# KUIS-AI-Tekalp-Research-Group/video-compression

Measured on AMD Instinct MI355X. Metric: frames/sec + bpp/PSNR on UVG 1080p GOP-8, 1/2/4/8 MI355X, higher is better.
Workload: dtype f32; 1 GPU; LHBDC 1080p GOP-8 inference, single lambda: 7 B-frames per GOP via Model.forward, 4 independent GOP(s) per GPU per step, hierarchy levels batched across them; gop=8, resolution=1920x1080, precision=fp32, parallelism=gop-shard x1, launch=hip-graph per GOP pass

## Files before the change

include/vc_hip.h:

```cpp
#ifndef VC_HIP_H
#define VC_HIP_H

#include <stddef.h>
#include <stdint.h>

#ifdef __cplusplus
extern "C" {
#endif

#define VC_OK 0
#define VC_EINVAL (-1)
#define VC_ELAUNCH (-2)
#define VC_ENOMEM (-3)
#define VC_EDATA (-4)

typedef void *vc_stream;

typedef struct {
    float *p;
    int n, h, w, c;
    long long sn, sh, sw;
} vc_view;

const char *vc_version(void);
// ... 115 lines not shown
int vc_gc_forward(vc_stream s, vc_view y, vc_view scales, vc_view means, const float *in_gain,
                  const float *out_gain, vc_view y_hat, double *bits_partial, int bits_slots,
                  const float *sym_src_p, int32_t *symbols, int32_t *indexes, const float *scale_table,
                  int n_scales, float *likelihoods);
int vc_gc_indexes(vc_stream s, vc_view scales, const float *scale_table, int n_scales, int32_t *indexes);
int vc_refine_scales(vc_stream s, vc_view scales, vc_view in, const float *w_oihw, const float *bias, const float *scale_table,
                     int n_scales, float rel_eps, int *counter);
int vc_gc_dequant(vc_stream s, const int32_t *symbols, vc_view means, const float *out_gain, vc_view y_hat);
typedef struct vc_refine_layer {
    vc_view in;
    const float *w_oihw;
    const float *bias;
    int k, stride, c0;
} vc_refine_layer;
int vc_refine_y_symbols(vc_stream s, vc_view y, vc_refine_layer y_layer, vc_view means, vc_refine_layer mu_layer, float eps,
                        int32_t *symbols, vc_view y_hat, const float *out_gain, int *counter);
int vc_refine_z_symbols(vc_stream s, vc_view z, vc_refine_layer z_layer, const float *eb_params, const float *in_gain, float eps,
                        int32_t *symbols, vc_view z_hat, const float *out_gain, int *counter);
int vc_bits_reduce(vc_stream s, const double *partial, int slots, int count, double *out);
int vc_bits_slots(void);
int vc_psnr_uint8(vc_stream s, const float *a_chw, const float *b_chw, int channels, int H, int W, int h, int w,
                  double *scratch, int slots, double *psnr_out);
size_t vc_msssim_workspace_bytes(int n, int channels, int h, int w);
int vc_msssim(vc_stream s, const float *a, const float *b, int n, int channels, int H, int W, int h, int w,
              long long image_pitch, int quantize, void *workspace, size_t workspace_bytes, double *terms_out,
              double *msssim_out);

int vc_pmf_to_quantized_cdf(const float *pmf, int n, int precision, uint32_t *cdf_out );
size_t vc_rans_bound(size_t count);
long long vc_rans_encode_with_indexes(const int32_t *symbols, const int32_t *indexes, size_t count,
                                      const int32_t *cdfs, int n_tables, int cdf_stride, const int32_t *cdf_sizes,
                                      const int32_t *offsets, uint8_t *out, size_t out_cap);
int vc_rans_decode_with_indexes(const uint8_t *data, size_t nbytes, const int32_t *indexes, size_t count,
                                const int32_t *cdfs, int n_tables, int cdf_stride, const int32_t *cdf_sizes,
                                const int32_t *offsets, int32_t *symbols_out);
int vc_rans_decode_stream(const uint8_t *data, size_t nbytes, uint64_t *state, const int32_t *indexes, size_t count,
                          const int32_t *cdfs, int n_tables, int cdf_stride, const int32_t *cdf_sizes,
                          const int32_t *offsets, int32_t *symbols_out);

int vc_gdn(vc_stream s, vc_view x, const float *gamma_packed, const float *beta_packed, int inverse, vc_view res ,
           vc_view out);
int vc_spynet_level(vc_stream s, vc_view first, vc_view second, vc_view flow_coarse, vc_view feat8, vc_view up2);
int vc_pool(vc_stream s, vc_view in, vc_view out, int k, float scale);
int vc_upsample(vc_stream s, vc_view in, vc_view out, int factor, int align_corners, float scale);
int vc_pad(vc_stream s, vc_view in, vc_view out);
int vc_blend(vc_stream s, vc_view fwbw, vc_view mask, vc_view cur, vc_view pred, vc_view resid);
int vc_factorized_bits(vc_stream s, vc_view z, const float *params, const float *in_gain, const float *out_gain,
                       vc_view z_hat, int32_t *symbols, double *bits_partial, int bits_slots, float *likelihoods);
int vc_gaussian_symbols(vc_stream s, vc_view y, vc_view scales, vc_view means, const float *in_gain,
                        const float *out_gain, vc_view y_hat, double *bits_partial, int bits_slots,
                        const float *sym_src_p, int32_t *symbols, int32_t *indexes, const float *scale_table,
                        int n_scales, float *likelihoods);

#ifdef __cplusplus
}
#endif
#endif
```

video-compression_amd/csrc/conv_api.hip:

```cpp
#include <stdlib.h>
#include <string.h>
#include "conv_mfma.h"

static inline int cfg_nt(int cfg) { return cfg == VC_CFG_N4 ? 4 : (cfg == VC_CFG_N16 ? 16 : 32); }
static inline int cfg_ks(int cfg) { return cfg == VC_CFG_N4 ? 4 : (cfg == VC_CFG_N16 ? 16 : 8); }
static inline int cfg_bn(int cfg)
{
    switch (cfg) {
    case VC_CFG_N128:
    case VC_CFG_N128B: return 128;
    case VC_CFG_N64: return 64;
    case VC_CFG_N32:
    case VC_CFG_N32T16: return 32;
    case VC_CFG_N4: return 4;
    default: return 16;
    }
}
static inline int round_up(int a, int b) { return (a + b - 1) / b * b; }

extern "C" int vc_conv_select_cfg(int cout, int cin, int k, int stride)
{
    (void)cin;
    int cfg;
    if (cout <= 4 && stride == 1 && (k == 3 || k == 5 || k == 7)) cfg = VC_CFG_N4;
// ... 197 lines not shown
    if (a.res_f16 && (!f16 || !d->res || !((d->cfg & 0xff) == VC_CFG_PWS || (d->cfg & 0xff) == VC_CFG_DMA))) return VC_EINVAL;
    a.res_first = (d->cfg & VC_CFG_RES_FIRST) ? 1 : 0;
    if (a.res_first && (!d->res || d->epi != VC_EPI_NONE || d->act == VC_ACT_SIGMOID || d->act == VC_ACT_CLAMP01)) return VC_EINVAL;
    a.cin_pad = round_up(a.Cin, f16 ? 2 * ck : ck);
    const int cfg0 = d->cfg & 0xff;
    const int th = (cfg0 == VC_CFG_N32T16) ? 16 : 8, tw = (cfg0 == VC_CFG_N4) ? 64 : 32;
    a.tiles_x = (a.Wo + tw - 1) / tw;
    a.tiles_y = (a.Ho + th - 1) / th;
    int cfg = d->cfg & 0xff;
    const bool exact = (d->cfg & VC_CFG_EXACT) != 0;
    while (!exact && (cfg == VC_CFG_N128 || cfg == VC_CFG_N64) &&
           (long long)a.tiles_x * a.tiles_y * a.N * (round_up(a.Cout, cfg_bn(cfg)) / cfg_bn(cfg)) < 512 &&
           vc_conv_chunk(cfg + 1, k, st, d->in.c) == ck)
        ++cfg;
    const int bn = cfg_bn(cfg);
    a.nblks = round_up(a.Cout, bn) / bn;
    a.total_blocks = a.tiles_x * a.tiles_y * a.nblks * a.N;
    {
        static const int band = [] { const char *e = getenv("VC_TILE_BAND"); const int v = e ? atoi(e) : 8; return v >= 1 ? v : 8; }();
        a.tile_band = band;
    }
    a.act = d->act; a.slope = d->slope;
    a.epi = d->epi; a.in_xform = d->in_xform; a.out_mode = d->out_mode;
    a.vec4 = ((a.Cin % 4) == 0 && (a.in_sw % 4) == 0 && (a.in_sh % 4) == 0 && (a.in_sn % 4) == 0 &&
              ((uintptr_t)a.in % 16) == 0) ? 1 : 0;
    if (a.in_f16)
        a.vec4 = ((a.Cin % 8) == 0 && (a.in_sw % 8) == 0 && (a.in_sh % 8) == 0 && (a.in_sn % 8) == 0 &&
                  ((uintptr_t)a.in % 16) == 0) ? 1 : 0;
    {
        auto ok = [](const void *ptr, long long sn, long long sh, long long sw) {
            return !ptr || (((uintptr_t)ptr % 16) == 0 && (sn % 4) == 0 && (sh % 4) == 0 && (sw % 4) == 0);
        };
        const int cgrp = (d->out_mode == VC_OUT_PIXELSHUFFLE2) ? (a.Cout >> 2) : a.Cout;
        a.vec_out = (cgrp % 4) == 0 && (a.out_sp3 ? ((uintptr_t)a.out % 16) == 0 : ok(a.out, a.out_sn, a.out_sh, a.out_sw)) &&
                    (a.res_sp3 ? ((uintptr_t)a.res % 8) == 0 : ok(a.res, a.res_sn, a.res_sh, a.res_sw)) &&
                    ok(a.mul, a.mul_sn, a.mul_sh, a.mul_sw) && ok(a.chscale, 0, 0, 0);
    }
    if (a.total_blocks <= 0) return VC_EINVAL;
    if (a.out_sp3 && !a.vec_out) return VC_EINVAL;
    if (f16 && !a.vec4) return VC_EINVAL;
    hipStream_t stream = as_stream(s);
    if (cfg == VC_CFG_PW) {
        if (!conv_pw_eligible(a, k, st, f16)) return VC_EINVAL;
        return conv_dispatch_pw(stream, a, f16);
    }
    if (cfg == VC_CFG_PWS) {
        if (!conv_pws_eligible(a, k, st, f16)) return VC_EINVAL;
        return conv_dispatch_pws(stream, a, f16);
    }
    if (cfg == VC_CFG_SPLIT)
        return conv_dispatch_split(stream, a, k, st);
    if (cfg == VC_CFG_DMA)
        return conv_dispatch_dma(stream, a, k, st, f16);
    switch (k) {
    case 1: return f16 ? conv_dispatch_k1_f16(stream, a, st, cfg, ck) : conv_dispatch_k1_f32(stream, a, st, cfg, ck);
    case 3: return f16 ? conv_dispatch_k3_f16(stream, a, st, cfg, ck) : conv_dispatch_k3_f32(stream, a, st, cfg, ck);
    case 5: return f16 ? conv_dispatch_k5_f16(stream, a, st, cfg, ck) : conv_dispatch_k5_f32(stream, a, st, cfg, ck);
    case 7: return f16 ? conv_dispatch_k7_f16(stream, a, st, cfg, ck) : conv_dispatch_k7_f32(stream, a, st, cfg, ck);
    }
    return VC_EINVAL;
}

#ifdef VC_STAMPS
extern "C" int vc_debug_read_stamps(unsigned long long *out8)
{
    if (hipDeviceSynchronize() != hipSuccess) return VC_ELAUNCH;
    if (hipMemcpyFromSymbol(out8, HIP_SYMBOL(g_vc_stamps), 8 * sizeof(unsigned long long)) != hipSuccess) return VC_ELAUNCH;
    unsigned long long zero[8] = {0};
    if (hipMemcpyToSymbol(HIP_SYMBOL(g_vc_stamps), zero, sizeof(zero)) != hipSuccess) return VC_ELAUNCH;
    return VC_OK;
}
extern "C" int vc_debug_set_skip(int mask)
{
    if (hipDeviceSynchronize() != hipSuccess) return VC_ELAUNCH;
    return hipMemcpyToSymbol(HIP_SYMBOL(g_vc_skip), &mask, sizeof(mask)) == hipSuccess ? VC_OK : VC_ELAUNCH;
}
#endif
```

video-compression_amd/csrc/conv_mfma.h:

```cpp
#pragma once
#include "common.h"

#include <type_traits>
#include <utility>

__device__ __forceinline__ void vc_tile_xy(int t, int tiles_x, int tiles_y, int band_rows, int &tx, int &ty)
{
    const int per_band = band_rows * tiles_x;
    const int band = t / per_band, r = t - band * per_band;
    const int rows = min(band_rows, tiles_y - band * band_rows);
    tx = r / rows;
    ty = band * band_rows + (r - tx * rows);
}

template <int I, int N, class F> __device__ __forceinline__ void static_for(F &&f)
{
    if constexpr (I < N) {
        f(std::integral_constant<int, I>{});
        static_for<I + 1, N>(std::forward<F>(f));
    }
}

#ifdef VC_STAMPS
__device__ unsigned long long g_vc_stamps[8];
// ... 710 lines not shown
    } else {
        conv_epilogue<C, F16>(p, acc, nblk, wm, wn, lane, oy0, ox0, img);
    }
    VC_T(t_end);
    VC_ACC(4, t_end, t_loop_end);
    VC_ACC(5, t_end, t_start);
    VC_ACC(6, 1ull, 0ull);
}

template <int KH, int KW, int S, int CK, class C, bool F16 = false, bool BLDS = false> int launch_conv(hipStream_t st, const ConvArgs &a)
{
    typedef ConvGeom<KH, KW, S, CK, C> G;
    const size_t lds_bytes = (G::LDS_FLOATS + 4) * sizeof(float) +
                             (BLDS ? (size_t)KH * KW * (a.cin_pad / G::KS) * 64 : 0);
    auto kern = conv_mfma_kernel<KH, KW, S, CK, C, F16, BLDS>;
    static vc_lds_raised raised;
    if (!vc_raise_lds_limit(reinterpret_cast<const void *>(kern), lds_bytes, raised)) return VC_ELAUNCH;
    hipLaunchKernelGGL(kern, dim3(a.total_blocks), dim3(256), lds_bytes, st, a);
    return hipGetLastError() == hipSuccess ? VC_OK : VC_ELAUNCH;
}

#ifdef VC_TU_F16
template <int KH, int KW, int S, int CK, class C> int launch_conv_p(hipStream_t st, const ConvArgs &a)
{
    return launch_conv<KH, KW, S, CK, C, VC_TU_F16 != 0>(st, a);
}
template <int KH, int KW, int S, int CK> int launch_conv_n4(hipStream_t st, const ConvArgs &a)
{
#if VC_TU_F16
    return VC_EINVAL;
#else
    const char *force = getenv("VC_N4_GLOBAL_WEIGHTS");
    if ((size_t)KH * KW * (a.cin_pad / 4) * 64 <= 32 * 1024 && !(force && force[0] == '1'))
        return launch_conv<KH, KW, S, CK, CfgN4, false, true>(st, a);
    return launch_conv<KH, KW, S, CK, CfgN4, false>(st, a);
#endif
}
#if VC_TU_F16
#define VC_DISPATCH(k) conv_dispatch_##k##_f16
#else
#define VC_DISPATCH(k) conv_dispatch_##k##_f32
#endif
#endif

#define VC_DECLARE_DISPATCH(k)                                                             \
    int conv_dispatch_##k##_f32(hipStream_t st, const ConvArgs &a, int stride, int cfg, int ck); \
    int conv_dispatch_##k##_f16(hipStream_t st, const ConvArgs &a, int stride, int cfg, int ck);
bool conv_pw_eligible(const ConvArgs &a, int k, int stride, bool f16);
bool conv_pws_eligible(const ConvArgs &a, int k, int stride, bool f16);
int conv_dispatch_pws(hipStream_t st, const ConvArgs &a, bool f16);
int conv_dispatch_pw(hipStream_t st, const ConvArgs &a, bool f16);
int conv_dispatch_dma(hipStream_t st, ConvArgs a, int k, int stride, bool f16);
int conv_dispatch_split(hipStream_t st, ConvArgs a, int k, int stride);
VC_DECLARE_DISPATCH(k1)
VC_DECLARE_DISPATCH(k3)
VC_DECLARE_DISPATCH(k5)
VC_DECLARE_DISPATCH(k7)
```

video-compression_amd/vcamd/hip.py:

```python
import contextlib
import ctypes
import os

import numpy as np
import torch

_PKG_DIR = os.path.dirname(os.path.dirname(os.path.abspath(__file__)))
LIB_PATH = os.environ.get("VC_HIP_LIB") or os.path.join(_PKG_DIR, "libvc_hip.so")

VC_OK = 0
ABI_VERSION = 6
ACT_NONE, ACT_RELU, ACT_LRELU, ACT_SIGMOID, ACT_CLAMP01 = 0, 1, 2, 3, 4
EPI_NONE, EPI_GDN, EPI_IGDN = 0, 1, 2
IN_NONE, IN_SQUARE = 0, 1
OUT_PLAIN, OUT_PIXELSHUFFLE2 = 0, 1
WARP_W1, WARP_W2, WARP_W3 = 1, 2, 3
EB_PARAMS_PER_CHANNEL = 60

_ERR = {-1: "VC_EINVAL (bad argument / unsupported shape)", -2: "VC_ELAUNCH (HIP launch failure)",
        -3: "VC_ENOMEM", -4: "VC_EDATA (corrupt bitstream / degenerate pmf)"}


class VcError(RuntimeError):
    pass
# ... 101 lines not shown
    sig("vc_split3", ci, vp, View, vp, cll)
    sig("vc_split3_pad", ci, vp, View, vp, cll, ci)
    sig("vc_nchw_to_nhwc", ci, vp, vp, View)
    sig("vc_nhwc_to_nchw", ci, vp, View, vp)
    sig("vc_u8hwc_to_f32nchw_pad", ci, vp, vp, ci, ci, vp, ci, ci)
    sig("vc_f32nchw_to_u8hwc", ci, vp, vp, ci, ci, vp, ci, ci)
    sig("vc_avgpool_reflectpad", ci, vp, View, View, ci, cf)
    sig("vc_maxpool2", ci, vp, View, View)
    sig("vc_maxpool2_sp3", ci, vp, vp, cll, ci, ci, ci, ci, vp, cll)
    sig("vc_avgpool2_sp3", ci, vp, vp, cll, ci, ci, ci, ci, cf, vp, cll, View)
    sig("vc_upsample_bilinear_sp3", ci, vp, View, vp, cll, ci, ci, cf)
    sig("vc_upsample_bilinear", ci, vp, View, View, ci, ci, cf)
    sig("vc_axpby", ci, vp, View, View, View, cf, cf)
    sig("vc_clamp01", ci, vp, View, View)
    sig("vc_channel_scale", ci, vp, View, vp, View)
    sig("vc_warp", ci, vp, ci, View, View, View)
    sig("vc_spynet_preprocess", ci, vp, vp, View)
    sig("vc_spynet_level_input", ci, vp, View, View, View, View, View)
    sig("vc_spynet_level_input_sp3", ci, vp, View, View, View, vp, View)
    sig("vc_lhbdc_blend", ci, vp, View, View, View, View, View)
    sig("vc_flex_blend", ci, vp, View, View, View, View, View, View)
    sig("vc_flex_motion_split", ci, vp, View, View, View, cf)
    sig("vc_quantize_mask", ci, vp, View, View, vp, ci, ci)
    sig("vc_deform_pack_weights", ci, vp, ci, ci, ci, vp)
    sig("vc_deform_conv2d", ci, vp, View, View, View, vp, vp, ci, View)
    sig("vc_offset_diversity", ci, vp, View, View, View, View, View, View, cf, vp, vp, ci, View)
    sig("vc_offset_diversity_hx", ci, vp, View, View, View, View, View, View, cf, vp, vp, ci, View)
    sig("vc_to_half", ci, vp, View, vp)
    sig("vc_offset_diversity_hxp", ci, vp, View, View, View, View, View, View, cf, vp, vp, ci, View)
    sig("vc_to_half_planar", ci, vp, View, ci, vp)
    sig("vc_attention_gate", ci, vp, View, View, View, View)
    sig("vc_sse_clamp01", ci, vp, View, View, vp, ci)
    sig("vc_select_flow", ci, vp, vp, ci, ctypes.c_double, ctypes.POINTER(View), View, vp)
    sig("vc_eb_forward", ci, vp, View, vp, vp, vp, View, vp, vp, ci, vp)
    sig("vc_eb_dequant", ci, vp, vp, vp, vp, View)
    sig("vc_gc_forward", ci, vp, View, View, View, vp, vp, View, vp, ci, vp, vp, vp, vp, ci, vp)
    sig("vc_gc_indexes", ci, vp, View, vp, ci, vp)
    sig("vc_refine_scales", ci, vp, View, View, vp, vp, vp, ci, cf, vp)
    sig("vc_gc_dequant", ci, vp, vp, View, vp, View)
    sig("vc_refine_y_symbols", ci, vp, View, RefineLayer, View, RefineLayer, cf, vp, View, vp, vp)
    sig("vc_refine_z_symbols", ci, vp, View, RefineLayer, vp, vp, cf, vp, View, vp, vp)
    sig("vc_bits_reduce", ci, vp, vp, ci, ci, vp)
    sig("vc_bits_slots", ci)
    sig("vc_psnr_uint8", ci, vp, vp, vp, ci, ci, ci, ci, ci, vp, ci, vp)
    sig("vc_msssim_workspace_bytes", sz, ci, ci, ci, ci)
    sig("vc_msssim", ci, vp, vp, vp, ci, ci, ci, ci, ci, ci, cll, ci, vp, sz, vp, vp)
    sig("vc_gdn", ci, vp, View, vp, vp, ci, View, View)
    sig("vc_pad", ci, vp, View, View)
    sig("vc_pmf_to_quantized_cdf", ci, vp, ci, ci, vp)
    sig("vc_rans_bound", sz, sz)
    sig("vc_rans_encode_with_indexes", cll, vp, vp, sz, vp, ci, ci, vp, vp, vp, sz)
    sig("vc_rans_decode_with_indexes", ci, vp, sz, vp, sz, vp, ci, ci, vp, vp, vp)
    sig("vc_rans_decode_stream", ci, vp, sz, vp, vp, sz, vp, ci, ci, vp, vp, vp)
    _lib = L
    return L


EXPORTED_SYMBOLS = [
    "vc_version", "vc_abi_version", "vc_target_arch", "vc_conv_select_cfg", "vc_conv_chunk", "vc_conv_packed_weight_floats",
    "vc_conv_packed_bias_floats", "vc_conv_pack_weights", "vc_conv_packed_weight_bytes_f16",
    "vc_conv_pack_weights_f16", "vc_conv_pack_tail_f16", "vc_conv2d_nhwc", "vc_conv_packed_weight_bytes_split",
    "vc_conv_pack_weights_split", "vc_split3", "vc_split3_pad", "vc_nchw_to_nhwc",
    "vc_nhwc_to_nchw", "vc_u8hwc_to_f32nchw_pad", "vc_f32nchw_to_u8hwc", "vc_avgpool_reflectpad", "vc_maxpool2", "vc_maxpool2_sp3", "vc_avgpool2_sp3", "vc_upsample_bilinear", "vc_upsample_bilinear_sp3", "vc_axpby", "vc_clamp01", "vc_channel_scale", "vc_warp",
    "vc_spynet_preprocess", "vc_spynet_level_input", "vc_spynet_level_input_sp3", "vc_lhbdc_blend", "vc_flex_blend",
    "vc_flex_motion_split", "vc_quantize_mask", "vc_deform_pack_weights", "vc_deform_conv2d", "vc_offset_diversity", "vc_offset_diversity_hx", "vc_to_half", "vc_offset_diversity_hxp", "vc_to_half_planar",
    "vc_attention_gate", "vc_sse_clamp01", "vc_select_flow", "vc_eb_forward", "vc_eb_dequant", "vc_gc_forward", "vc_gc_indexes", "vc_refine_scales",
    "vc_refine_y_symbols", "vc_refine_z_symbols", "vc_gc_dequant", "vc_bits_reduce", "vc_bits_slots", "vc_psnr_uint8", "vc_msssim_workspace_bytes", "vc_msssim", "vc_pmf_to_quantized_cdf", "vc_rans_bound",
    "vc_rans_encode_with_indexes", "vc_rans_decode_with_indexes", "vc_rans_decode_stream",
    "vc_gdn", "vc_spynet_level", "vc_pool", "vc_upsample", "vc_pad", "vc_blend", "vc_factorized_bits", "vc_gaussian_symbols",
]


DEBUG_SYNC = bool(int(os.environ.get("VC_DEBUG_SYNC", "0")))


def check(rc, what):
    if rc != VC_OK:
        raise VcError(f"{what} failed: {_ERR.get(rc, rc)}")
    if DEBUG_SYNC:
        try:
            torch.cuda.synchronize()
        except Exception as e:
            raise VcError(f"device fault during {what}: {e}") from e


def stream():
    return ctypes.c_void_p(torch.cuda.current_stream().cuda_stream)


class T:
    __slots__ = ("buf", "n", "h", "w", "c", "sn", "sh", "sw", "off", "dtype")

    def __init__(self, buf, n, h, w, c, sn, sh, sw, off=0, dtype="f32"):
        self.buf, self.n, self.h, self.w, self.c = buf, n, h, w, c
        self.sn, self.sh, self.sw, self.off, self.dtype = sn, sh, sw, off, dtype

    @staticmethod
    def empty(n, h, w, c, device, dtype="f32"):
        if dtype == "sp3":
            if c % 8:
                raise VcError("a split tensor holds groups of 8 channels")
            return T(torch.empty(n * h * w * c * 3, dtype=torch.int16, device=device), n, h, w, c, c // 8, 0, 0, 0, dtype)
        buf = torch.empty(n * h * w * c, dtype=torch.float16 if dtype == "f16" else torch.float32, device=device)
        return T(buf, n, h, w, c, h * w * c, w * c, c, 0, dtype)

    def channels(self, c0, c1):
        if self.dtype == "sp3":
            if c0 % 8 or c1 % 8:
                raise VcError("a split tensor is sliced in groups of 8 channels")
            return T(self.buf, self.n, self.h, self.w, c1 - c0, self.sn, 0, 0, self.off + c0 // 8, self.dtype)
        return T(self.buf, self.n, self.h, self.w, c1 - c0, self.sn, self.sh, self.sw, self.off + c0, self.dtype)

    def crop(self, h, w):
        if self.dtype == "sp3":
            raise VcError("a split tensor is plane-major: it has no crop window")
        return T(self.buf, self.n, h, w, self.c, self.sn, self.sh, self.sw, self.off, self.dtype)

    def images(self, n0, n1):
        if self.dtype == "sp3":
            return T(self.buf, n1 - n0, self.h, self.w, self.c, self.sn, 0, 0, self.off + n0 * self.sn, self.dtype)
        return T(self.buf, n1 - n0, self.h, self.w, self.c, self.sn, self.sh, self.sw, self.off + n0 * self.sn, self.dtype)

# ... 407 lines not shown
        if chscale is not None:
            d.chscale = chscale.data_ptr()
        d.kh = d.kw = self.k
        d.stride = self.stride
        d.act, d.slope = act, slope
        d.epi, d.in_xform = epi, in_xform
        d.out_mode = OUT_PIXELSHUFFLE2 if self.ps else OUT_PLAIN
        d.cfg = self.cfg
        flags = (CFG_RES_FIRST if res_first else 0) | (CFG_OUT_SP3 if sp_out else 0)
        if use16:
            d.wpk = self.wpk16.data_ptr()
            flags |= CFG_F16 | (CFG_IN_F16 if half_in else 0) | (CFG_OUT_F16 if half_out else 0) | (CFG_RES_F16 if res_half else 0)
        key = (x.n, x.h, x.w, flags) if (act < ACT_SIGMOID and epi == EPI_NONE) else (x.n, x.h, x.w, flags, act, epi)
        pack = CFG_PACK128 if self.cfg == 0 else 0
        if gdn_half:
            flags |= CFG_OUT_F16
            d.cfg = CFG_PWS | CFG_EXACT | flags
        elif tail is not None:
            tw, tb = tail.tail_pack()
            d.tail_wpk, d.tail_bias = tw.data_ptr(), tb.data_ptr()
            d.cfg = CFG_DMA | CFG_EXACT | flags | pack
        else:
            d.cfg = self._pick_cfg(d, key, flags | pack) | pack
        what = f"vc_conv2d_nhwc(k={self.k},s={self.stride},{self.cin}->{self.cout}{'+1x1 tail' if tail is not None else ''})"

        def launch_once():
            rc = lib().vc_conv2d_nhwc(stream(), ctypes.byref(d))
            if rc == -1 and tail is None and (d.cfg & 0xff) != self.cfg:
                d.cfg = self.cfg | (d.cfg & ~0x1ff)
                rc = lib().vc_conv2d_nhwc(stream(), ctypes.byref(d))
            return rc
        if timer is None:
            check(launch_once(), what)
        else:
            hq, wq = (ho // 2, wo // 2) if self.ps else (ho, wo)
            flops = 2.0 * x.n * hq * wq * self.cout * (self.cin * self.k * self.k + (tail.cin if tail is not None else 0))
            key = f"conv k{self.k}{'+k1' if tail is not None else ''} s{self.stride} {self.cin}->{self.cout} @{x.n}x{x.h}x{x.w}"
            nbytes = (x.n * x.h * x.w * self.cin * (2 if half_in else 4) + x.n * ho * wo * co * (2 if half_out else 4)
                      + self.cout * self.cin * self.k * self.k * (2 if use16 else 4)
                      + (x.n * ho * wo * co * (2 if res_half else 4) if res is not None else 0) + (x.n * ho * wo * co * 4 if mul is not None else 0))
            c0 = d.cfg & 0xff
            if c0 == CFG_DMA:
                kernel_symbols[key] = f"conv_dma_kernel<DmaCfg<{self.k}, {self.k}, {self.cin // (32 if use16 else 16)},"
            elif c0 == CFG_PWS:
                kernel_symbols[key] = "conv_pws_kernel<"
            elif c0 == 7:
                kernel_symbols[key] = f"conv_mfma_kernel<{self.k}, {self.k}, 1, 16, TileCfg<32, 16"
            else:
                kernel_symbols[key] = f"conv_mfma_kernel<{self.k}, {self.k}, {self.stride},"
            timer.bracket(key, flops, lambda: check(launch_once(), what), nbytes)
        return out


def avgpool_reflectpad(x, k, scale=1.0, out_h=None, out_w=None):
    hp, wp = x.h // k, x.w // k
    out = T.empty(x.n, out_h or hp, out_w or wp, x.c, x.buf.device)
    check(lib().vc_avgpool_reflectpad(stream(), x.view(), out.view(), k, scale), "vc_avgpool_reflectpad")
    return out


def avgpool2_split(x, out_sp3):
    out = T.empty(x.n, x.h // 2, x.w // 2, x.c, x.buf.device, "sp3" if out_sp3 else "f32")
    timed_hbm(f"k_avgpool2_sp3 c{x.c} @{x.n}x{x.h}x{x.w}", x.n * x.c * (6.0 * x.h * x.w + (6.0 if out_sp3 else 4.0) * out.h * out.w),
              lambda: check(lib().vc_avgpool2_sp3(stream(), x.ptr, x.image_bytes, x.n, x.h, x.w, x.c, 1.0, out.ptr if out_sp3 else None,
                                                  out.image_bytes if out_sp3 else 0, NULL_VIEW if out_sp3 else out.view()), "vc_avgpool2_sp3"))
    return out


def maxpool2(x):
    if x.dtype == "sp3":
        out = T.empty(x.n, x.h // 2, x.w // 2, x.c, x.buf.device, "sp3")
        timed_hbm(f"k_maxpool2_sp3 c{x.c} @{x.n}x{x.h}x{x.w}", 6.0 * x.n * x.c * (x.h * x.w + out.h * out.w),
                  lambda: check(lib().vc_maxpool2_sp3(stream(), x.ptr, x.image_bytes, x.n, x.h, x.w, x.c, out.ptr, out.image_bytes), "vc_maxpool2_sp3"))
        return out
    out = T.empty(x.n, x.h // 2, x.w // 2, x.c, x.buf.device)
    check(lib().vc_maxpool2(stream(), x.view(), out.view()), "vc_maxpool2")
    return out


def upsample_bilinear(x, factor, align_corners=False, scale=1.0, out=None):
    if out is None:
        out = T.empty(x.n, x.h * factor, x.w * factor, x.c, x.buf.device)
    if out.dtype == "sp3":
        timed_hbm(f"k_upsample_bilinear_sp3 x{factor} c{x.c} @{x.n}x{x.h}x{x.w}", x.n * x.c * (4.0 * x.h * x.w + 6.0 * out.h * out.w),
                  lambda: check(lib().vc_upsample_bilinear_sp3(stream(), x.view(), out.ptr, out.image_bytes, factor, int(align_corners), scale),
                                "vc_upsample_bilinear_sp3"))
        return out
    timed_hbm(f"k_upsample_bilinear x{factor} c{x.c} @{x.n}x{x.h}x{x.w}", 4.0 * x.n * x.c * (x.h * x.w + out.h * out.w),
              lambda: check(lib().vc_upsample_bilinear(stream(), x.view(), out.view(), factor, int(align_corners), scale),
                            "vc_upsample_bilinear"))
    return out


def axpby(a, b, alpha=1.0, beta=1.0, out=None):
    if out is None:
        out = T.empty(a.n, a.h, a.w, a.c, a.buf.device)
    check(lib().vc_axpby(stream(), a.view(), b.view() if b is not None else NULL_VIEW, out.view(), alpha, beta),
          "vc_axpby")
    return out


def to_half(x):
    out = T.empty(x.n, x.h, x.w, x.c, x.buf.device, "f16")
    check(lib().vc_to_half(stream(), x.view(), out.ptr), "vc_to_half")
    return out

# ... 237 lines not shown
```

video-compression_amd/vcamd/layers.py:

```python
import math

import numpy as np
import scipy.stats
import torch
import torch.nn as nn
import torch.nn.functional as F

from . import hip
from .hip import T


class LowerBound(nn.Module):
    def __init__(self, bound):
        super().__init__()
        self.register_buffer("bound", torch.Tensor([float(bound)]))


class NonNegativeParametrizer(nn.Module):
    def __init__(self, minimum=0.0, reparam_offset=2 ** -18):
        super().__init__()
        pedestal = float(reparam_offset) ** 2
        self.register_buffer("pedestal", torch.Tensor([pedestal]))
        self.lower_bound = LowerBound((float(minimum) + pedestal) ** 0.5)

# ... 42 lines not shown
        self.gamma = nn.Parameter(self.gamma_reparam.init(gamma_init * torch.eye(in_channels)))

    def run(self, x, res=None, out=None, out_sp3=False, out_f16=False):
        if self._packed is None:
            with torch.no_grad():
                c = self.beta.numel()
                beta = self.beta_reparam.resolve(self.beta)
                gamma = self.gamma_reparam.resolve(self.gamma).reshape(c, c, 1, 1)
            self._packed = hip.PackedConv(gamma, beta, device=self.beta.device)
        return self._packed(x, out=out, epi=hip.EPI_IGDN if self.inverse else hip.EPI_GDN, mul=x,
                            in_xform=hip.IN_SQUARE, res=res, out_sp3=out_sp3, out_f16=out_f16)


def conv3x3(in_ch, out_ch, stride=1):
    return nn.Conv2d(in_ch, out_ch, kernel_size=3, stride=stride, padding=1)


def conv1x1(in_ch, out_ch, stride=1):
    return nn.Conv2d(in_ch, out_ch, kernel_size=1, stride=stride)


def subpel_conv3x3(in_ch, out_ch, r=1):
    return nn.Sequential(nn.Conv2d(in_ch, out_ch * r ** 2, kernel_size=3, padding=1), nn.PixelShuffle(r))


class ResidualBlockWithStride(_Prepared):
    def __init__(self, in_ch, out_ch, stride=2):
        super().__init__()
        self.conv1 = conv3x3(in_ch, out_ch, stride=stride)
        self.leaky_relu = nn.LeakyReLU(inplace=True)
        self.conv2 = conv3x3(out_ch, out_ch)
        self.gdn = GDN(out_ch)
        self.skip = conv1x1(in_ch, out_ch, stride=stride) if (stride != 1 or in_ch != out_ch) else None

    def out_hw(self, h, w):
        s = self.conv1.stride[0]
        return (h - 1) // s + 1, (w - 1) // s + 1

    def _pack(self):
        if self._packed is None:
            self._packed = (pack_conv(self.conv1), pack_conv(self.conv2),
                            pack_conv(self.skip) if self.skip is not None else None)
        return self._packed

    def half_stream_ok(self):
        c1, _, sk = self._pack()
        return hip.HALF_RESIDUAL and hip.HALF_ACTIVATIONS and c1.half_ok and sk is not None and sk.half_ok

    def run(self, x, out=None, out_sp3=False, out_f16=False):
        c1, c2, sk = self._pack()
        if x.dtype == "f16" and not self.half_stream_ok():
            raise hip.VcError("a half-precision tensor reached a residual block that reads its input in fp32")
        ho, wo = self.out_hw(x.h, x.w)
        t = c1(x, act=hip.ACT_LRELU, slope=0.01, out_f16=c2.half_ok, out_sp3=hip.wants_split(c2, x, ho, wo))
        u = c2(t)
        identity = x if sk is None else sk(x)
        return self.gdn.run(u, res=identity, out=out, out_sp3=out_sp3, out_f16=out_f16)


class ResidualBlockUpsample(_Prepared):
    def __init__(self, in_ch, out_ch, upsample=2):
        super().__init__()
        self.subpel_conv = subpel_conv3x3(in_ch, out_ch, upsample)
        self.leaky_relu = nn.LeakyReLU(inplace=True)
        self.conv = conv3x3(out_ch, out_ch)
        self.igdn = GDN(out_ch, inverse=True)
        self.upsample = subpel_conv3x3(in_ch, out_ch, upsample)

    def _pack(self):
        if self._packed is None:
            self._packed = (pack_conv(self.subpel_conv[0], pixelshuffle=True), pack_conv(self.conv),
                            pack_conv(self.upsample[0], pixelshuffle=True))
        return self._packed

    def out_hw(self, h, w):
        return 2 * h, 2 * w

    def split_in_ok(self, n, h, w):
        sp, _, up = self._pack()
        return hip.wants_split_at(sp, n, h, w) and hip.wants_split_at(up, n, h, w)

    def half_stream_ok(self):
        sp, _, up = self._pack()
        return hip.HALF_RESIDUAL and hip.HALF_ACTIVATIONS and sp.half_ok and up.half_ok

    def run(self, x, out=None, out_sp3=False, out_f16=False):
        sp, cv, up = self._pack()
        if x.dtype == "f16" and not self.half_stream_ok():
            raise hip.VcError("a half-precision tensor reached a residual block that reads its input in fp32")
        xs = x
        if x.dtype == "f32" and self.split_in_ok(x.n, x.h, x.w):
            xs = hip.split3(x)
        t = sp(xs, act=hip.ACT_LRELU, slope=0.01, out_f16=cv.half_ok,
               out_sp3=hip.wants_split(cv, x, 2 * x.h, 2 * x.w))
        u = cv(t)
        identity = up(xs)
        return self.igdn.run(u, res=identity, out=out, out_sp3=out_sp3, out_f16=out_f16)


class ResidualBlock(_Prepared):
    def __init__(self, in_ch, out_ch):
        super().__init__()
        self.conv1 = conv3x3(in_ch, out_ch)
        self.leaky_relu = nn.LeakyReLU(inplace=True)
        self.conv2 = conv3x3(out_ch, out_ch)
        self.skip = conv1x1(in_ch, out_ch) if in_ch != out_ch else None
# ... 600 lines not shown
```

Before: 21.85 frames/s.

## Add thin-channel conv head kernels and fused stride-2 stem conv+skip pair

Adds a dedicated CUDA-core kernel for thin output heads (7x7 16->2 and 5x5 32->1 convs), which previously went through the MFMA N4 path. It also adds a fused kernel that computes a residual block's 3x3 stride-2 conv (with leaky ReLU) and its 1x1 stride-2 skip conv from a single read of the input, for inputs with 4 or fewer channels and 128 output channels. The aim is to avoid MFMA tiles that are mostly wasted on tiny channel counts and to cut one pass over the input plus one launch. Both paths are on by default and can be turned off with VC_THIN=0. The cost is extra code paths that must match the existing conv numerics.

Result: no change. 21.84 frames/s, median of 2 (-0.1%).

```diff
diff --git a/include/vc_hip.h b/include/vc_hip.h
--- a/include/vc_hip.h
+++ b/include/vc_hip.h
@@ -191,6 +191,10 @@
                         const float *sym_src_p, int32_t *symbols, int32_t *indexes, const float *scale_table,
                         int n_scales, float *likelihoods);
 
+int vc_conv_thin_enabled(void);
+int vc_conv_stem_pair(vc_stream s, vc_view in, const float *w_a, const float *bias_a, const float *w_b, const float *bias_b, float slope,
+                      vc_view out_a, void *out_a_split, long long out_a_image_bytes, vc_view out_b);
+
 #ifdef __cplusplus
 }
 #endif
diff --git a/video-compression_amd/csrc/conv_api.hip b/video-compression_amd/csrc/conv_api.hip
--- a/video-compression_amd/csrc/conv_api.hip
+++ b/video-compression_amd/csrc/conv_api.hip
@@ -273,6 +273,10 @@
         return conv_dispatch_split(stream, a, k, st);
     if (cfg == VC_CFG_DMA)
         return conv_dispatch_dma(stream, a, k, st, f16);
+    if (!f16 && !exact) {
+        const int rc = conv_dispatch_thin_head(stream, a, k, st, cfg);
+        if (rc != VC_THIN_NOT_SERVED) return rc;
+    }
     switch (k) {
     case 1: return f16 ? conv_dispatch_k1_f16(stream, a, st, cfg, ck) : conv_dispatch_k1_f32(stream, a, st, cfg, ck);
     case 3: return f16 ? conv_dispatch_k3_f16(stream, a, st, cfg, ck) : conv_dispatch_k3_f32(stream, a, st, cfg, ck);
diff --git a/video-compression_amd/csrc/conv_mfma.h b/video-compression_amd/csrc/conv_mfma.h
--- a/video-compression_amd/csrc/conv_mfma.h
+++ b/video-compression_amd/csrc/conv_mfma.h
@@ -786,6 +786,8 @@
 int conv_dispatch_pw(hipStream_t st, const ConvArgs &a, bool f16);
 int conv_dispatch_dma(hipStream_t st, ConvArgs a, int k, int stride, bool f16);
 int conv_dispatch_split(hipStream_t st, ConvArgs a, int k, int stride);
+constexpr int VC_THIN_NOT_SERVED = 1;
+int conv_dispatch_thin_head(hipStream_t st, const ConvArgs &a, int k, int stride, int cfg);
 VC_DECLARE_DISPATCH(k1)
 VC_DECLARE_DISPATCH(k3)
 VC_DECLARE_DISPATCH(k5)
diff --git a/video-compression_amd/csrc/conv_thin.hip b/video-compression_amd/csrc/conv_thin.hip
--- /dev/null
+++ b/video-compression_amd/csrc/conv_thin.hip
@@ -0,0 +1,353 @@
+#include <stdlib.h>
+#include "conv_mfma.h"
+
+extern "C" int vc_conv_thin_enabled(void)
+{
+    static const int on = [] { const char *e = getenv("VC_THIN"); return (e && e[0] == '0' && e[1] == 0) ? 0 : 1; }();
+    return on;
+}
+
+constexpr int THIN_P = 3, THIN_LX = 16, THIN_TW = THIN_P * THIN_LX;
+
+template <int K, int CIN> struct ThinHeadGeom {
+    static constexpr int C4 = CIN / 4;
+    static constexpr int COLS = THIN_TW + K - 1;
+    static constexpr int COLSP = COLS | 1;
+    static constexpr size_t lds_bytes(int th, int cout) { return ((size_t)(th + K - 1) * C4 * COLSP + (size_t)K * K * C4 * cout) * 16; }
+};
+
+struct ThinHeadArgs {
+    const float *in;
+    long long in_sn, in_sh, in_sw;
+    int N, H, W;
+    float *out;
+    long long out_sn, out_sh, out_sw;
+    const float *res;
+    long long res_sn, res_sh, res_sw;
+    const float *wpk;
+    const float *bias;
+    int act;
+    int vec2;
+    int tiles_x, tiles_y;
+};
+
+template <int K, int CIN, int COUT, int TH>
+__global__ __launch_bounds__(THIN_LX *TH) void k_conv_thin_head(ThinHeadArgs a)
+{
+    typedef ThinHeadGeom<K, CIN> G;
+    constexpr int C4 = G::C4, COLS = G::COLS, COLSP = G::COLSP, ROWS = TH + K - 1, P = THIN_P, NT = THIN_LX * TH, SEG = P + K - 1;
+    extern __shared__ __attribute__((aligned(16))) unsigned char thin_smem[];
+    f32x4 *tile = reinterpret_cast<f32x4 *>(thin_smem);
+    f32x4 *wl = tile + ROWS * C4 * COLSP;
+    const int tid = threadIdx.x;
+    const int bid = blockIdx.x;
+    const int tx = bid % a.tiles_x, ty = (bid / a.tiles_x) % a.tiles_y, img = bid / (a.tiles_x * a.tiles_y);
+    const int x0 = tx * THIN_TW, y0 = ty * TH;
+
+    for (int i = tid; i < K * K * C4 * COUT; i += NT) {
+        const int co = i % COUT, c4 = (i / COUT) % C4, tap = i / (COUT * C4);
+        wl[i] = *reinterpret_cast<const f32x4 *>(a.wpk + ((size_t)(tap * C4 + c4) * 64 + co) * 4);
+    }
+    const float *inb = a.in + (long long)img * a.in_sn;
+    for (int i = tid; i < ROWS * COLS * C4; i += NT) {
+        const int c4 = i % C4, col = (i / C4) % COLS, row = i / (C4 * COLS);
+        const int iy = y0 - K / 2 + row, ix = x0 - K / 2 + col;
+        f32x4 v = {0.f, 0.f, 0.f, 0.f};
+        if (iy >= 0 && iy < a.H && ix >= 0 && ix < a.W)
+            v = *reinterpret_cast<const f32x4 *>(inb + (long long)iy * a.in_sh + (long long)ix * a.in_sw + 4 * c4);
+        tile[(row * C4 + c4) * COLSP + col] = v;
+    }
+    __syncthreads();
+
+    const int lx = tid % THIN_LX, ly = tid / THIN_LX;
+    float acc[P][COUT];
+#pragma unroll
+    for (int p = 0; p < P; ++p)
+#pragma unroll
+        for (int co = 0; co < COUT; ++co) acc[p][co] = 0.0f;
+
+#pragma unroll 1
+    for (int ky = 0; ky < K; ++ky) {
+        f32x4 seg[SEG][C4];
+        const f32x4 *rowp = tile + (ly + ky) * C4 * COLSP + lx * P;
+#pragma unroll
+        for (int c4 = 0; c4 < C4; ++c4)
+#pragma unroll
+            for (int j = 0; j < SEG; ++j) seg[j][c4] = rowp[c4 * COLSP + j];
+        const f32x4 *wrow = wl + ky * K * C4 * COUT;
+#pragma unroll
+        for (int kx = 0; kx < K; ++kx)
+#pragma unroll
+            for (int c4 = 0; c4 < C4; ++c4) {
+                f32x4 w[COUT];
+#pragma unroll
+                for (int co = 0; co < COUT; ++co) w[co] = wrow[(kx * C4 + c4) * COUT + co];
+#pragma unroll
+                for (int e = 0; e < 4; ++e)
+#pragma unroll
+                    for (int p = 0; p < P; ++p)
+#pragma unroll
+                        for (int co = 0; co < COUT; ++co) acc[p][co] = fmaf(seg[p + kx][c4][e], w[co][e], acc[p][co]);
+            }
+    }
+
+    const int oy = y0 + ly;
+    if (oy >= a.H) return;
+    float b[COUT];
+#pragma unroll
+    for (int co = 0; co < COUT; ++co) b[co] = a.bias[co];
+#pragma unroll
+    for (int p = 0; p < P; ++p) {
+        const int ox = x0 + lx * P + p;
+        if (ox >= a.W) continue;
+        float v[COUT];
+#pragma unroll
+        for (int co = 0; co < COUT; ++co) v[co] = acc[p][co] + b[co];
+        const long long o_off = (long long)img * a.out_sn + (long long)oy * a.out_sh + (long long)ox * a.out_sw;
+        if (a.res) {
+            const float *r = a.res + (long long)img * a.res_sn + (long long)oy * a.res_sh + (long long)ox * a.res_sw;
+            if (COUT == 2 && a.vec2) {
+                const float2 rv = *reinterpret_cast<const float2 *>(r);
+                v[0] += rv.x;
+                v[COUT - 1] += rv.y;
+            } else {
+#pragma unroll
+                for (int co = 0; co < COUT; ++co) v[co] += r[co];
+            }
+        }
+        if (a.act == VC_ACT_SIGMOID) {
+#pragma unroll
+            for (int co = 0; co < COUT; ++co) v[co] = 1.0f / (1.0f + expf(-v[co]));
+        }
+        if (COUT == 2 && a.vec2) {
+            *reinterpret_cast<float2 *>(a.out + o_off) = make_float2(v[0], v[COUT - 1]);
+        } else {
+#pragma unroll
+            for (int co = 0; co < COUT; ++co) a.out[o_off + co] = v[co];
+        }
+    }
+}
+
+template <int K, int CIN, int COUT, int TH> static int launch_thin_head(hipStream_t st, ThinHeadArgs a)
+{
+    typedef ThinHeadGeom<K, CIN> G;
+    static vc_lds_raised raised;
+    const size_t lds = G::lds_bytes(TH, COUT);
+    auto kern = k_conv_thin_head<K, CIN, COUT, TH>;
+    if (!vc_raise_lds_limit(reinterpret_cast<const void *>(kern), lds, raised)) return VC_ELAUNCH;
+    a.tiles_x = (a.W + THIN_TW - 1) / THIN_TW;
+    a.tiles_y = (a.H + TH - 1) / TH;
+    const long long blocks = (long long)a.tiles_x * a.tiles_y * a.N;
+    if (blocks <= 0 || blocks > 0x7fffffffLL) return VC_EINVAL;
+    hipLaunchKernelGGL(kern, dim3((unsigned)blocks), dim3(THIN_LX * TH), lds, st, a);
+    VC_LAUNCH_CHECK();
+    return VC_OK;
+}
+
+int conv_dispatch_thin_head(hipStream_t st, const ConvArgs &a, int k, int stride, int cfg)
+{
+    if (!vc_conv_thin_enabled()) return VC_THIN_NOT_SERVED;
+    const bool shape7 = k == 7 && a.Cin == 16 && a.Cout == 2, shape5 = k == 5 && a.Cin == 32 && a.Cout == 1;
+    if (cfg != VC_CFG_N4 || stride != 1 || !(shape7 || shape5) || a.cin_pad != a.Cin) return VC_THIN_NOT_SERVED;
+    if (a.epi != VC_EPI_NONE || a.in_xform != VC_IN_NONE || a.out_mode != VC_OUT_PLAIN || a.mul || a.chscale || a.res_first || a.tail_wpk ||
+        a.in_f16 || a.out_f16 || a.res_f16 || a.in_sp3 || a.out_sp3 || a.res_sp3)
+        return VC_THIN_NOT_SERVED;
+    if (!(a.act == VC_ACT_NONE || (a.act == VC_ACT_SIGMOID && !a.res))) return VC_THIN_NOT_SERVED;
+    if (!a.vec4 || ((uintptr_t)a.wpk % 16) != 0 || ((uintptr_t)a.bias % 4) != 0) return VC_THIN_NOT_SERVED;
+    if (a.Ho != a.H || a.Wo != a.W) return VC_THIN_NOT_SERVED;
+    ThinHeadArgs t;
+    t.in = a.in; t.in_sn = a.in_sn; t.in_sh = a.in_sh; t.in_sw = a.in_sw;
+    t.N = a.N; t.H = a.H; t.W = a.W;
+    t.out = a.out; t.out_sn = a.out_sn; t.out_sh = a.out_sh; t.out_sw = a.out_sw;
+    t.res = a.res; t.res_sn = a.res_sn; t.res_sh = a.res_sh; t.res_sw = a.res_sw;
+    t.wpk = a.wpk; t.bias = a.bias; t.act = a.act;
+    auto even = [](const void *p, long long sn, long long sh, long long sw) {
+        return !p || (((uintptr_t)p % 8) == 0 && (sn % 2) == 0 && (sh % 2) == 0 && (sw % 2) == 0);
+    };
+    t.vec2 = (a.Cout == 2 && even(a.out, a.out_sn, a.out_sh, a.out_sw) && even(a.res, a.res_sn, a.res_sh, a.res_sw)) ? 1 : 0;
+    t.tiles_x = t.tiles_y = 0;
+    const long long tiles_x = (a.W + THIN_TW - 1) / THIN_TW;
+    if (shape7) {
+        if (tiles_x * ((a.H + 31) / 32) * a.N >= 512) return launch_thin_head<7, 16, 2, 32>(st, t);
+        return launch_thin_head<7, 16, 2, 8>(st, t);
+    }
+    if (tiles_x * ((a.H + 15) / 16) * a.N >= 512) return launch_thin_head<5, 32, 1, 16>(st, t);
+    return launch_thin_head<5, 32, 1, 8>(st, t);
+}
+
+constexpr int STEM_COUT = 128, STEM_RUN = 64, STEM_COLS = 2 * STEM_RUN + 1;
+
+struct ThinStemArgs {
+    const float *in;
+    long long in_sn, in_sh, in_sw;
+    int N, H, W, Ho, Wo;
+    const float *wa, *ba, *wb, *bb;
+    float slope;
+    float *out_a;
+    long long a_sn, a_sh, a_sw;
+    unsigned char *out_a_split;
+    long long a_image_bytes;
+    float *out_b;
+    long long b_sn, b_sh, b_sw;
+    int runs_x;
+    long long total_runs;
+};
+
+template <int CIN> __global__ __launch_bounds__(256) void k_conv_thin_stem(ThinStemArgs a)
+{
+    constexpr int KA = 9 * CIN;
+    __shared__ __attribute__((aligned(16))) float wa_l[KA][STEM_COUT];
+    __shared__ __attribute__((aligned(16))) float wb_l[CIN][STEM_COUT];
+    __shared__ __attribute__((aligned(16))) float ba_l[STEM_COUT], bb_l[STEM_COUT];
+    __shared__ float in_l[3][STEM_COLS][CIN];
+    __shared__ __attribute__((aligned(16))) unsigned char rec_l[VC_RECORDS_LDS(16)];
+    const int tid = threadIdx.x;
+    for (int i = tid; i < KA * STEM_COUT; i += 256) {
+        const int co = i % STEM_COUT, k = i / STEM_COUT, ci = k % CIN, tap = k / CIN;
+        wa_l[k][co] = a.wa[((size_t)co * CIN + ci) * 9 + tap];
+    }
+    for (int i = tid; i < CIN * STEM_COUT; i += 256) wb_l[i / STEM_COUT][i % STEM_COUT] = a.wb[(size_t)(i % STEM_COUT) * CIN + i / STEM_COUT];
+    if (tid < STEM_COUT) {
+        ba_l[tid] = a.ba ? a.ba[tid] : 0.0f;
+        bb_l[tid] = a.bb ? a.bb[tid] : 0.0f;
+    }
+    const int j16 = tid % 16, px = tid / 16;
+    const bool split = a.out_a_split != nullptr;
+    const int swp = split ? (j16 >> 3) : 0;
+    const int cha0 = split ? 8 * j16 + 4 * swp : 4 * j16, cha1 = split ? 8 * j16 + 4 - 4 * swp : 64 + 4 * j16;
+    const int chb0 = 4 * j16, chb1 = 64 + 4 * j16;
+    const long long plane_bytes = (long long)a.Ho * a.Wo * 48;
+
+    for (long long run = blockIdx.x; run < a.total_runs; run += gridDim.x) {
+        const int rx = (int)(run % a.runs_x);
+        const long long t = run / a.runs_x;
+        const int oy = (int)(t % a.Ho), img = (int)(t / a.Ho);
+        const int ox0 = rx * STEM_RUN;
+        __syncthreads();
+        const float *inb = a.in + (long long)img * a.in_sn;
+        for (int i = tid; i < 3 * STEM_COLS * CIN; i += 256) {
+            const int ci = i % CIN, col = (i / CIN) % STEM_COLS, r = i / (CIN * STEM_COLS);
+            const int iy = 2 * oy - 1 + r, ix = 2 * ox0 - 1 + col;
+            float v = 0.0f;
+            if (iy >= 0 && iy < a.H && ix >= 0 && ix < a.W) v = inb[(long long)iy * a.in_sh + (long long)ix * a.in_sw + ci];
+            in_l[r][col][ci] = v;
+        }
+        __syncthreads();
+
+        f32x4 acc0[4], acc1[4];
+#pragma unroll
+        for (int q = 0; q < 4; ++q) acc0[q] = acc1[q] = f32x4{0.f, 0.f, 0.f, 0.f};
+#pragma unroll 1
+        for (int tap = 0; tap < 9; ++tap) {
+            const int ky = tap / 3, kx = tap - 3 * ky;
+#pragma unroll
+                for (int ci = 0; ci < CIN; ++ci) {
+                    const int k = tap * CIN + ci;
+                    const f32x4 w0 = *reinterpret_cast<const f32x4 *>(&wa_l[k][cha0]);
+                    const f32x4 w1 = *reinterpret_cast<const f32x4 *>(&wa_l[k][cha1]);
+#pragma unroll
+                    for (int q = 0; q < 4; ++q) {
+                        const float x = in_l[ky][2 * (px + 16 * q) + kx][ci];
+#pragma unroll
+                        for (int e = 0; e < 4; ++e) {
+                            acc0[q][e] = fmaf(x, w0[e], acc0[q][e]);
+                            acc1[q][e] = fmaf(x, w1[e], acc1[q][e]);
+                        }
+                    }
+                }
+        }
+        {
+            const f32x4 b0 = *reinterpret_cast<const f32x4 *>(&ba_l[cha0]), b1 = *reinterpret_cast<const f32x4 *>(&ba_l[cha1]);
+#pragma unroll
+            for (int q = 0; q < 4; ++q) {
+                f32x4 v0 = acc0[q] + b0, v1 = acc1[q] + b1;
+#pragma unroll
+                for (int e = 0; e < 4; ++e) {
+                    v0[e] = v0[e] >= 0.0f ? v0[e] : v0[e] * a.slope;
+                    v1[e] = v1[e] >= 0.0f ? v1[e] : v1[e] * a.slope;
+                }
+                const int ox = ox0 + px + 16 * q;
+                if (split) {
+                    vc_u32x4 ph, pm, pl;
+                    vc_split_record(swp ? v1 : v0, swp ? v0 : v1, ph, pm, pl);
+                    const int oxq = ox0 + 16 * q;
+                    const int npx = min(16, a.Wo - oxq);
+                    unsigned char *dst0 = a.out_a_split + (long long)img * a.a_image_bytes + ((long long)oy * a.Wo + oxq) * 48;
+                    if (q) __syncthreads();
+                    vc_store_records_256<16>(rec_l, tid, ox < a.Wo, ph, pm, pl, dst0, plane_bytes, npx);
+                } else if (ox < a.Wo) {
+                    float *o = a.out_a + (long long)img * a.a_sn + (long long)oy * a.a_sh + (long long)ox * a.a_sw;
+                    *reinterpret_cast<f32x4 *>(o + cha0) = v0;
+                    *reinterpret_cast<f32x4 *>(o + cha1) = v1;
+                }
+            }
+        }
+
+#pragma unroll
+        for (int q = 0; q < 4; ++q) acc0[q] = acc1[q] = f32x4{0.f, 0.f, 0.f, 0.f};
+#pragma unroll
+        for (int ci = 0; ci < CIN; ++ci) {
+            const f32x4 w0 = *reinterpret_cast<const f32x4 *>(&wb_l[ci][chb0]);
+            const f32x4 w1 = *reinterpret_cast<const f32x4 *>(&wb_l[ci][chb1]);
+#pragma unroll
+            for (int q = 0; q < 4; ++q) {
+                const float x = in_l[1][2 * (px + 16 * q) + 1][ci];
+#pragma unroll
+                for (int e = 0; e < 4; ++e) {
+                    acc0[q][e] = fmaf(x, w0[e], acc0[q][e]);
+                    acc1[q][e] = fmaf(x, w1[e], acc1[q][e]);
+                }
+            }
+        }
+        {
+            const f32x4 b0 = *reinterpret_cast<const f32x4 *>(&bb_l[chb0]), b1 = *reinterpret_cast<const f32x4 *>(&bb_l[chb1]);
+#pragma unroll
+            for (int q = 0; q < 4; ++q) {
+                const int ox = ox0 + px + 16 * q;
+                if (ox < a.Wo) {
+                    float *o = a.out_b + (long long)img * a.b_sn + (long long)oy * a.b_sh + (long long)ox * a.b_sw;
+                    *reinterpret_cast<f32x4 *>(o + chb0) = acc0[q] + b0;
+                    *reinterpret_cast<f32x4 *>(o + chb1) = acc1[q] + b1;
+                }
+            }
+        }
+    }
+}
+
+extern "C" int vc_conv_stem_pair(vc_stream s, vc_view in, const float *w_a, const float *bias_a, const float *w_b, const float *bias_b,
+                                 float slope, vc_view out_a, void *out_a_split, long long out_a_image_bytes, vc_view out_b)
+{
+    if (!in.p || !w_a || !w_b || !out_b.p) return VC_EINVAL;
+    if (in.c < 1 || in.c > 4 || in.n < 1 || in.h < 1 || in.w < 1) return VC_EINVAL;
+    if ((out_a.p != nullptr) == (out_a_split != nullptr)) return VC_EINVAL;
+    const int ho = (in.h - 1) / 2 + 1, wo = (in.w - 1) / 2 + 1;
+    auto view_ok = [&](const vc_view &v) {
+        return v.n == in.n && v.h == ho && v.w == wo && v.c == STEM_COUT && ((uintptr_t)v.p % 16) == 0 && (v.sn % 4) == 0 && (v.sh % 4) == 0 &&
+               (v.sw % 4) == 0;
+    };
+    if (!view_ok(out_b)) return VC_EINVAL;
+    if (out_a.p && !view_ok(out_a)) return VC_EINVAL;
+    if (((uintptr_t)w_a % 4) || ((uintptr_t)w_b % 4) || ((uintptr_t)bias_a % 4) || ((uintptr_t)bias_b % 4) || ((uintptr_t)in.p % 4)) return VC_EINVAL;
+    ThinStemArgs a;
+    a.in = in.p; a.in_sn = in.sn; a.in_sh = in.sh; a.in_sw = in.sw;
+    a.N = in.n; a.H = in.h; a.W = in.w; a.Ho = ho; a.Wo = wo;
+    a.wa = w_a; a.ba = bias_a; a.wb = w_b; a.bb = bias_b; a.slope = slope;
+    a.out_a = out_a.p; a.a_sn = out_a.sn; a.a_sh = out_a.sh; a.a_sw = out_a.sw;
+    a.out_a_split = static_cast<unsigned char *>(out_a_split);
+    a.a_image_bytes = out_a_image_bytes ? out_a_image_bytes : (long long)(STEM_COUT / 8) * ho * wo * 48;
+    if (out_a_split && (((uintptr_t)out_a_split % 16) || (a.a_image_bytes % 16) || a.a_image_bytes < (long long)(STEM_COUT / 8) * ho * wo * 48))
+        return VC_EINVAL;
+    a.out_b = out_b.p; a.b_sn = out_b.sn; a.b_sh = out_b.sh; a.b_sw = out_b.sw;
+    a.runs_x = (wo + STEM_RUN - 1) / STEM_RUN;
+    a.total_runs = (long long)a.runs_x * ho * in.n;
+    const int grid = (int)(a.total_runs < 256 * 4 ? a.total_runs : 256 * 4);
+    hipStream_t st = as_stream(s);
+    switch (in.c) {
+    case 1: hipLaunchKernelGGL(k_conv_thin_stem<1>, dim3(grid), dim3(256), 0, st, a); break;
+    case 2: hipLaunchKernelGGL(k_conv_thin_stem<2>, dim3(grid), dim3(256), 0, st, a); break;
+    case 3: hipLaunchKernelGGL(k_conv_thin_stem<3>, dim3(grid), dim3(256), 0, st, a); break;
+    default: hipLaunchKernelGGL(k_conv_thin_stem<4>, dim3(grid), dim3(256), 0, st, a); break;
+    }
+    VC_LAUNCH_CHECK();
+    return VC_OK;
+}
diff --git a/video-compression_amd/vcamd/hip.py b/video-compression_amd/vcamd/hip.py
--- a/video-compression_amd/vcamd/hip.py
+++ b/video-compression_amd/vcamd/hip.py
@@ -177,6 +177,8 @@
     sig("vc_rans_encode_with_indexes", cll, vp, vp, sz, vp, ci, ci, vp, vp, vp, sz)
     sig("vc_rans_decode_with_indexes", ci, vp, sz, vp, sz, vp, ci, ci, vp, vp, vp)
     sig("vc_rans_decode_stream", ci, vp, sz, vp, vp, sz, vp, ci, ci, vp, vp, vp)
+    sig("vc_conv_thin_enabled", ci)
+    sig("vc_conv_stem_pair", ci, vp, View, vp, vp, vp, vp, cf, View, vp, cll, View)
     _lib = L
     return L
 
@@ -193,6 +195,7 @@
     "vc_refine_y_symbols", "vc_refine_z_symbols", "vc_gc_dequant", "vc_bits_reduce", "vc_bits_slots", "vc_psnr_uint8", "vc_msssim_workspace_bytes", "vc_msssim", "vc_pmf_to_quantized_cdf", "vc_rans_bound",
     "vc_rans_encode_with_indexes", "vc_rans_decode_with_indexes", "vc_rans_decode_stream",
     "vc_gdn", "vc_spynet_level", "vc_pool", "vc_upsample", "vc_pad", "vc_blend", "vc_factorized_bits", "vc_gaussian_symbols",
+    "vc_conv_thin_enabled", "vc_conv_stem_pair",
 ]
 
 
@@ -706,6 +709,32 @@
         return out
 
 
+def thin_enabled():
+    return bool(lib().vc_conv_thin_enabled())
+
+
+def conv_stem_pair(x, conv1, skip, slope, out_sp3=False):
+    ws = [p.detach() if p is not None else None for p in (conv1.weight, conv1.bias, skip.weight, skip.bias)]
+    if any(w is not None and (w.dtype != torch.float32 or not w.is_contiguous() or w.device != x.buf.device) for w in ws):
+        raise VcError("vc_conv_stem_pair reads contiguous fp32 weights on the input's device")
+    ho, wo, co = (x.h - 1) // 2 + 1, (x.w - 1) // 2 + 1, conv1.out_channels
+    t = T.empty(x.n, ho, wo, co, x.buf.device, "sp3" if out_sp3 else "f32")
+    identity = T.empty(x.n, ho, wo, co, x.buf.device)
+    ptr = [None if w is None else w.data_ptr() for w in ws]
+
+    def launch():
+        check(lib().vc_conv_stem_pair(stream(), x.view(), ptr[0], ptr[1], ptr[2], ptr[3], slope, NULL_VIEW if out_sp3 else t.view(),
+                                      t.ptr if out_sp3 else None, t.image_bytes if out_sp3 else 0, identity.view()), "vc_conv_stem_pair")
+    if timer is None:
+        launch()
+    else:
+        key = f"conv k3+k1 s2 {x.c}->{co} pair @{x.n}x{x.h}x{x.w}"
+        kernel_symbols[key] = f"k_conv_thin_stem<{x.c}>"
+        timer.bracket(key, 2.0 * x.n * ho * wo * co * x.c * 10, launch,
+                      x.n * x.h * x.w * x.c * 4 + x.n * ho * wo * co * ((6 if out_sp3 else 4) + 4) + co * x.c * 10 * 4)
+    return t, identity
+
+
 def avgpool_reflectpad(x, k, scale=1.0, out_h=None, out_w=None):
     hp, wp = x.h // k, x.w // k
     out = T.empty(x.n, out_h or hp, out_w or wp, x.c, x.buf.device)
diff --git a/video-compression_amd/vcamd/layers.py b/video-compression_amd/vcamd/layers.py
--- a/video-compression_amd/vcamd/layers.py
+++ b/video-compression_amd/vcamd/layers.py
@@ -118,6 +118,10 @@
         if x.dtype == "f16" and not self.half_stream_ok():
             raise hip.VcError("a half-precision tensor reached a residual block that reads its input in fp32")
         ho, wo = self.out_hw(x.h, x.w)
+        if (sk is not None and self.conv1.in_channels <= 4 and self.conv1.out_channels == 128 and self.conv1.stride[0] == 2
+                and x.dtype == "f32" and not c1.half_ok and hip.thin_enabled()):
+            t, identity = hip.conv_stem_pair(x, self.conv1, self.skip, 0.01, out_sp3=hip.wants_split(c2, x, ho, wo))
+            return self.gdn.run(c2(t), res=identity, out=out, out_sp3=out_sp3, out_f16=out_f16)
         t = c1(x, act=hip.ACT_LRELU, slope=0.01, out_f16=c2.half_ok, out_sp3=hip.wants_split(c2, x, ho, wo))
         u = c2(t)
         identity = x if sk is None else sk(x)
```
